# jamie8johnson/cqs

Measured on AMD Instinct MI355X. Metric: queries/sec @k=20 (brute-force cosine scan + top-k, 768-d fp32), higher is better.
Workload: dtype f32; 1 GPU; BASELINE configs[1]: 1000000 x 768 fp32 unit vectors, 1 query per step, brute-force cosine top-20; mode=single, rows_per_gpu=1000000, total_rows=1000000, dim=768, k=20, parallelism=single GPU, ranks_seen=1

## Files before the change

cqs_amd/csrc/index.hip:

```cpp
#include <hip/hip_runtime.h>

#include <algorithm>
#include <cstdio>
#include <cstdlib>
#include <cstring>
#include <new>

#include "abi_guard.h"
#include "roctx.h"
#include "index_internal.h"
#include "scan_bf16.h"
#include "scan_i8.h"
#include "search_host.h"

using cqs::kMaxK;
using cqs::kRowsPerBlock;

namespace cqs_idx {

uint64_t pad_rows(uint64_t n) { return (n + kRowsPerBlock - 1) / kRowsPerBlock * kRowsPerBlock; }

int32_t fail(cqs_hip_index* idx, int32_t code, const char* what, hipError_t e) {
    char buf[512];
    if (e != hipSuccess)
// ... 348 lines not shown
    if (x->done) hipEventDestroy(x->done);
    if (x->stream) hipStreamDestroy(x->stream);
    delete x;
} CQS_ABI_CATCH_VOID

uint64_t cqs_hip_index_len(const cqs_hip_index* x) CQS_ABI_TRY { return x ? (x->sh ? cqs_sharded::len(x) : x->n) : 0; } CQS_ABI_CATCH_VAL(0)
uint32_t cqs_hip_index_dim(const cqs_hip_index* x) CQS_ABI_TRY { return x ? x->dim : 0; } CQS_ABI_CATCH_VAL(0)
uint32_t cqs_hip_index_metric(const cqs_hip_index* x) CQS_ABI_TRY { return x ? x->metric : 0; } CQS_ABI_CATCH_VAL(0)
uint32_t cqs_hip_index_max_k(const cqs_hip_index* x) CQS_ABI_TRY { (void)x; return kMaxK; } CQS_ABI_CATCH_VAL(0)
int32_t cqs_hip_index_poisoned(const cqs_hip_index* x) CQS_ABI_TRY {
    if (x && x->sh) return cqs_sharded::poisoned(x);
    return x && x->poisoned.load(std::memory_order_acquire) ? 1 : 0;
} CQS_ABI_CATCH_NOHANDLE
int32_t cqs_hip_index_device(const cqs_hip_index* x) CQS_ABI_TRY { return x ? x->device : -1; } CQS_ABI_CATCH_NOHANDLE
uint64_t cqs_hip_index_row_base(const cqs_hip_index* x) CQS_ABI_TRY { return x ? x->row_base : 0; } CQS_ABI_CATCH_VAL(0)

size_t cqs_hip_index_last_error(const cqs_hip_index* x, char* buf, size_t cap) CQS_ABI_TRY {
    if (!x || !buf || cap == 0) return 0;
    std::lock_guard<std::mutex> g(x->mu);
    return cqs_search::copy_last_error(x->last_error.data(), x->last_error.size(), buf, cap);
} CQS_ABI_CATCH_VAL(0)

void cqs_hip_unpack_keys(const uint64_t* keys, size_t count, uint64_t* rows, float* scores) CQS_ABI_TRY {
    cqs_search::unpack_keys(keys, count, rows, scores);
} CQS_ABI_CATCH_VOID

size_t cqs_hip_merge_keys(const uint64_t* lists, const uint32_t* counts, size_t n_lists, size_t stride, size_t k,
                          uint64_t* out_keys) CQS_ABI_TRY {
    return cqs_search::merge_keys(lists, counts, n_lists, stride, k, out_keys);
} CQS_ABI_CATCH_VAL(0)

int32_t cqs_hip_index_search_device(cqs_hip_index* x, const float* d_queries, uint32_t b, uint32_t k,
                                    const uint32_t* d_keep_bitset, uint32_t mode, float threshold,
                                    uint64_t* d_out_keys, uint32_t* d_out_counts, void* stream) CQS_ABI_TRY {
    CQS_ROCTX_RANGE("cqs_hip_index_search_device");
    if (!x) return CQS_HIP_ERR_INVALID;
    if (x->sh) return CQS_HIP_ERR_INVALID;
    std::lock_guard<std::mutex> g(x->mu);
    if (x->poisoned.load(std::memory_order_acquire)) return CQS_HIP_ERR_POISONED;
    if (b == 0) return CQS_HIP_OK;
    if (!d_queries || !d_out_keys || !d_out_counts) return fail(x, CQS_HIP_ERR_INVALID, "search_device: null buffer");
    if (k == 0 || k > kMaxK) return fail(x, CQS_HIP_ERR_INVALID, "search_device: k out of range");
    if (mode > CQS_HIP_MODE_PIPELINE) return fail(x, CQS_HIP_ERR_INVALID, "search_device: bad mode");
    if (b > max_query_block(x)) return fail(x, CQS_HIP_ERR_INVALID, "search_device: batch exceeds scratch budget");
    HIP_TRY(x, hipSetDevice(x->device));
    hipStream_t st = (hipStream_t)stream;
    if (x->n == 0) {
        HIP_TRY(x, hipMemsetAsync(d_out_counts, 0, (size_t)b * sizeof(uint32_t), st));
        return CQS_HIP_OK;
    }
    int32_t rc = ensure_scratch(x, b, k);
    if (rc != CQS_HIP_OK) return rc;
    const uint32_t* gate = nullptr;
    if (shadow_takes(x, b, k, false) &&
        (rc = shadow_pass(x, d_queries, b, k, d_keep_bitset, mode, threshold, d_out_keys, d_out_counts, st, &gate)) != CQS_HIP_OK)
        return rc;
    return enqueue_search(x, d_queries, b, k, d_keep_bitset, mode, threshold, d_out_keys, d_out_counts, st, false, gate);
} CQS_ABI_CATCH(x)

}

namespace cqs_idx {

static void print_debug_stamps(cqs_hip_index* x) {
    unsigned long long h[16];
    if (hipMemcpy(h, x->d_dbg, sizeof h, hipMemcpyDeviceToHost) == hipSuccess)
        fprintf(stderr, "[cqs_hip] select_finish us: zero %.2f hist %.2f decide %.2f groups %.2f scores %.2f sort %.2f emit %.2f | groups=%llu cand=%llu\n",
                0.0, (h[1] - h[0]) / 100.0, (h[2] - h[1]) / 100.0, (h[3] - h[2]) / 100.0, (h[4] - h[3]) / 100.0,
                (h[5] - h[4]) / 100.0, (h[6] - h[5]) / 100.0, h[8], h[9]);
    std::vector<unsigned long long> w(2 * cqs::kDbgWaves);
    if (hipMemcpy(w.data(), x->d_dbg + 16, w.size() * sizeof(unsigned long long), hipMemcpyDeviceToHost) != hipSuccess) return;
    std::vector<double> st, en;
    unsigned long long t0 = ~0ull;
    for (uint32_t i = 0; i < cqs::kDbgWaves; ++i) if (w[2 * i] && w[2 * i] < t0) t0 = w[2 * i];
    for (uint32_t i = 0; i < cqs::kDbgWaves; ++i)
        if (w[2 * i] && w[2 * i + 1]) { st.push_back((w[2 * i] - t0) / 100.0); en.push_back((w[2 * i + 1] - t0) / 100.0); }
    if (!st.empty()) {
        std::sort(st.begin(), st.end());
        std::sort(en.begin(), en.end());
        auto pc = [](const std::vector<double>& v, double f) { return v[(size_t)(f * (v.size() - 1))]; };
        fprintf(stderr, "[cqs_hip] scan waves=%zu start us p0 %.1f p50 %.1f p90 %.1f p100 %.1f | end us p0 %.1f p10 %.1f p50 %.1f p90 %.1f p100 %.1f | select ends %.1f\n",
                st.size(), pc(st, 0), pc(st, .5), pc(st, .9), pc(st, 1), pc(en, 0), pc(en, .1), pc(en, .5), pc(en, .9), pc(en, 1),
                (h[6] - t0) / 100.0);
    }
    (void)hipMemset(x->d_dbg + 16, 0, w.size() * sizeof(unsigned long long));
}

static int32_t host_block(cqs_hip_index* x, const cqs_combine_req* const* qs, uint32_t nq, uint8_t* slots, uint32_t k,
                          const uint32_t* d_keep, uint32_t mode, float thr, bool gemv_only, std::vector<const cqs_combine_req*>* redo) {
    const KeepTab table{x->d_keep_tab, (uint32_t)x->keep_tab_stride, slots};
    const KeepTab* tab = slots ? &table : nullptr;
    HIP_TRY(x, hipMemcpyAsync(x->d_q, x->h_q, (size_t)nq * x->dim * sizeof(float), hipMemcpyHostToDevice, x->stream));
    const bool direct = x->h_out_keys_dev && x->h_out_counts_dev && (size_t)nq * k <= kDirectOutKeys;
    uint64_t* const keys = direct ? x->h_out_keys_dev : x->d_out_keys;
    uint32_t* const counts = direct ? x->h_out_counts_dev : x->d_out_counts;
    int32_t rc = redo ? shadow_pass(x, x->d_q, nq, k, d_keep, mode, thr, keys, counts, x->stream, nullptr, tab)
                      : enqueue_search(x, x->d_q, nq, k, d_keep, mode, thr, keys, counts, x->stream, gemv_only, nullptr, tab);
    if (rc != CQS_HIP_OK) return rc;
    if (redo) HIP_TRY(x, record_done(x, x->stream));
    if (!direct) {
        HIP_TRY(x, hipMemcpyAsync(x->h_out_keys, x->d_out_keys, (size_t)nq * k * sizeof(uint64_t), hipMemcpyDeviceToHost, x->stream));
        HIP_TRY(x, hipMemcpyAsync(x->h_out_counts, x->d_out_counts, (size_t)nq * sizeof(uint32_t), hipMemcpyDeviceToHost, x->stream));
    }
    const uint32_t* cert = nullptr;
    if (redo) HIP_TRY(x, shadow_verdicts(x, nq, &cert));
    HIP_TRY(x, hipStreamSynchronize(x->stream));
    if (!redo && x->d_dbg) print_debug_stamps(x);
    if (redo) redo->clear();
    uint64_t certified = 0;
// ... 251 lines not shown
```

cqs_amd/csrc/index_internal.h:

```cpp
#pragma once
#include <hip/hip_runtime.h>

#include <atomic>
#include <chrono>
#include <condition_variable>
#include <deque>
#include <mutex>
#include <string>
#include <vector>

#include "../../include/cqs_hip.h"
#include "scan_kernels.h"

namespace cqs_sharded { struct ShardSet; }
namespace cqs_idx { struct Shadow; }
namespace cqs_mmr { struct Scratch; }
namespace cqs_search { struct Args; }

struct cqs_combine_req {
    const float* q;
    uint32_t k, mode;
    float thr;
    uint64_t* out_rows;
    float* out_scores;
// ... 82 lines not shown

namespace cqs_idx {

constexpr size_t kMaxTimingEvents = 8192;
constexpr uint64_t kNtBytes = 200ull << 20;
constexpr uint32_t kGauxQueries = 32;
constexpr uint32_t kGauxMinK = 100;
constexpr uint32_t kCombineCap = 32;
constexpr size_t kDirectOutKeys = 8192;

uint64_t pad_rows(uint64_t n);
int32_t fail(cqs_hip_index* idx, int32_t code, const char* what, hipError_t e = hipSuccess);
void free_scratch(cqs_hip_index* x);
int32_t ensure_scratch(cqs_hip_index* x, uint32_t b, uint32_t k);
uint32_t max_query_block(const cqs_hip_index* x);
struct KeepTab { const uint32_t* d_tab; uint32_t stride; const uint8_t* slot; };
cqs::ScanArgs scan_args(const cqs_hip_index* x, const float* d_q, uint32_t b, uint32_t k, const uint32_t* d_keep,
                        uint32_t mode, float thr, size_t elem_bytes, bool gemv_only, void* dbg, const uint32_t* gate,
                        const KeepTab* tab = nullptr);
struct ShadowRows { const uint16_t* bf16; const int8_t* i8; const float* i8_scale; const float* bq; };
int32_t scan_select(cqs_hip_index* x, const cqs::ScanArgs& a, hipStream_t st, const ShadowRows* shadow,
                    uint64_t* out_keys, uint32_t* out_counts);
inline hipError_t order_after_last(cqs_hip_index* x, hipStream_t st) {
    return x->done_valid && x->done_stream != st ? hipStreamWaitEvent(st, x->done, 0) : hipSuccess;
}
inline hipError_t record_done(cqs_hip_index* x, hipStream_t st) {
    const hipError_t e = hipEventRecord(x->done, st);
    if (e == hipSuccess) { x->done_stream = st; x->done_valid = true; }
    return e;
}
int32_t enqueue_search(cqs_hip_index* x, const float* d_q, uint32_t b, uint32_t k, const uint32_t* d_keep,
                       uint32_t mode, float thr, uint64_t* d_out_keys, uint32_t* d_out_counts, hipStream_t st,
                       bool gemv_only = false, const uint32_t* gate = nullptr, const KeepTab* tab = nullptr);
hipError_t quiesce(cqs_hip_index* x);
int32_t create_owned(const float* rows, uint64_t n, uint32_t dim, uint32_t metric, int32_t device, uint64_t row_base,
                     cqs_hip_index** out);
int32_t stage_keep(cqs_hip_index* x, const uint32_t* host_words, uint64_t words);
int32_t ensure_keep(cqs_hip_index* x, uint64_t words);
bool ensure_keep_tab(cqs_hip_index* x);
void free_keep_tab(cqs_hip_index* x);
int32_t create_common(uint64_t n, uint32_t dim, uint32_t metric, int32_t device, uint64_t row_base,
                      cqs_hip_index** out, cqs_hip_index** made);
void read_combine_env(cqs_hip_index* x);
int32_t shadow_auto(cqs_hip_index* x);
int32_t shadow_extend(cqs_hip_index* x, uint64_t n_old);
void shadow_free(cqs_hip_index* x);
struct ShadowBuffers { uint16_t* bf16; int8_t* i8; float* i8_scale; };
ShadowBuffers shadow_buffers(const cqs_hip_index* x);
bool shadow_takes(const cqs_hip_index* x, uint32_t b, uint32_t k, bool gemv_only);
bool shadow_uses_i8(const cqs_hip_index* x, uint32_t b, uint32_t k);
int32_t shadow_pass(cqs_hip_index* x, const float* d_q, uint32_t nb, uint32_t k, const uint32_t* d_keep, uint32_t mode,
                    float thr, uint64_t* out_keys, uint32_t* out_counts, hipStream_t st, const uint32_t** device_gate,
                    const KeepTab* tab = nullptr);
hipError_t shadow_verdicts(cqs_hip_index* x, uint32_t nb, const uint32_t** h_cert);

bool search_planned(cqs_hip_index* x, const cqs_search::Args& a, int32_t* rc);
std::vector<cqs_combine_req> requests(const cqs_search::Args& a, float thr);
int32_t injected_failure(cqs_hip_index* x);
int32_t search_blocks_locked(cqs_hip_index* x, const cqs_combine_req* qs, uint32_t b, uint32_t k_eff, const uint32_t* d_keep,
                             uint32_t mode, float threshold, bool gemv_only);
void tags_free(cqs_hip_index* x);
void tags_regrow(cqs_hip_index* x);

int32_t search_host_locked(cqs_hip_index* x, const cqs_combine_req* qs, uint32_t b, uint32_t k, const uint32_t* keep_bitset,
                           uint32_t mode, float threshold, bool gemv_only);
int32_t search_filtered_locked(cqs_hip_index* x, const cqs_combine_req* qs, uint32_t b, uint32_t k, uint32_t mode, float threshold);
int32_t combine_search(cqs_hip_index* x, cqs_combine_req& r);

struct Segment { int device; float* d_rows; uint64_t rows; hipStream_t stream; };
int32_t save_segments(cqs_hip_index* err_owner, const std::vector<Segment>& segs, uint32_t dim, uint32_t metric,
                      const char* path, uint64_t* out_checksum);
int32_t open_blob(const char* path, uint32_t expected_dim, uint64_t expected_rows, int* fd_out, uint64_t* rows,
                  uint32_t* metric, uint64_t* checksum);
int32_t read_blob_into(int fd, uint64_t checksum, uint32_t dim, const std::vector<Segment>& segs);

}

namespace cqs_mmr {
void free_scratch(cqs_hip_index* x);
int32_t run(cqs_hip_index* owner, hipStream_t st, const float* src, const uint32_t* h_idx, const float* h_scores, uint32_t m,
            uint32_t limit, float lambda, float* out_gram, uint32_t* out_picks);
int32_t gather_rows(cqs_hip_index* c, const uint32_t* h_idx, uint32_t mc, const float** out_block);
int32_t staging(cqs_hip_index* parent, uint32_t m, float** out_block);
}

namespace cqs_sharded {
int32_t pairwise(cqs_hip_index* parent, const uint64_t* cand_rows, uint32_t m, float* out);
int32_t mmr(cqs_hip_index* parent, const uint64_t* cand_rows, const float* cand_scores, uint32_t m, uint32_t limit,
            float lambda, uint32_t* out_picks, uint32_t* out_count);
void destroy(cqs_hip_index* parent);
int32_t search(cqs_hip_index* parent, const float* queries, uint32_t b, uint32_t query_dim, uint32_t k,
               const uint32_t* keep_bitset, uint32_t mode, float threshold, uint64_t* out_rows, float* out_scores,
               uint32_t* out_counts);
int32_t search_combined(cqs_hip_index* parent, cqs_combine_req* const* batch, uint32_t nb);
int32_t neighbors(cqs_hip_index* parent, uint64_t target_row, uint32_t limit, uint64_t* out_rows, float* out_scores,
                  uint32_t* out_count);
int32_t extend(cqs_hip_index* parent, const float* rows, uint64_t n_new);
int32_t save(cqs_hip_index* parent, const char* path, uint64_t* out_checksum);
uint64_t len(const cqs_hip_index* parent);
int32_t poisoned(const cqs_hip_index* parent);
void set_timing(cqs_hip_index* parent, int32_t enable);
int32_t scan_time(cqs_hip_index* parent, uint32_t* launches, double* total_ms);
}

#define HIP_TRY(idx, expr)                                                        \
    do {                                                                          \
// ... 5 lines not shown
```

cqs_amd/csrc/index_shadow.hip:

```cpp
#include <cstdlib>
#include <cstring>
#include <new>

#include "abi_guard.h"
#include "index_internal.h"
#include "scan_bf16.h"
#include "scan_i8.h"

namespace cqs_idx {

constexpr uint64_t kShadowAutoBytes = 1ull << 30;
constexpr uint64_t kShadowFreeMinBytes = 4ull << 30;
constexpr double kShadowFreeFrac = 0.10;
constexpr uint32_t kStatWords = 10, kStatCounts = 3, kStatI8 = 5, kStatI8Counts = 8;

struct Shadow {
    uint16_t* d_bf16 = nullptr;
    uint64_t cap = 0;
    int8_t* d_i8 = nullptr;
    float* d_i8_scale = nullptr;
    double r8 = 0.0, norm8 = 0.0;
    double r = 0.0;
    double norm = 0.0;
    unsigned long long* d_stats = nullptr;
    uint64_t* d_ekeys = nullptr;
    uint32_t* d_cert = nullptr;
    float* d_bq = nullptr;
    uint32_t* d_tickets = nullptr;
    uint32_t* h_cert = nullptr;
    uint32_t* h_cert_dev = nullptr;
};

static void shadow_device_counts(cqs_hip_index* x, uint32_t first, uint64_t* certified, uint64_t* fallbacks) {
    unsigned long long c[2];
    if (!x->shadow || !x->shadow->d_stats || quiesce(x) != hipSuccess) return;
    hipError_t e = hipMemcpyAsync(c, x->shadow->d_stats + first, sizeof c, hipMemcpyDeviceToHost, x->stream);
    if (e == hipSuccess) e = hipStreamSynchronize(x->stream);
    if (e != hipSuccess) { (void)hipGetLastError(); return; }
    *certified += c[0];
    *fallbacks += c[1];
}

static void i8_free(Shadow* s) {
    hipFree(s->d_i8); hipFree(s->d_i8_scale);
    s->d_i8 = nullptr; s->d_i8_scale = nullptr;
}

void shadow_free(cqs_hip_index* x) {
    Shadow* s = x->shadow;
    if (!s) return;
    uint64_t c = 0, f = 0;
    shadow_device_counts(x, kStatCounts, &c, &f);
    x->stat_certified.fetch_add(c, std::memory_order_relaxed);
    x->stat_fallbacks.fetch_add(f, std::memory_order_relaxed);
    c = f = 0;
    shadow_device_counts(x, kStatI8Counts, &c, &f);
    x->stat_i8_certified.fetch_add(c, std::memory_order_relaxed);
    x->stat_i8_fallbacks.fetch_add(f, std::memory_order_relaxed);
    i8_free(s);
    hipFree(s->d_bf16); hipFree(s->d_stats); hipFree(s->d_ekeys);
    hipFree(s->d_cert); hipFree(s->d_bq); hipFree(s->d_tickets); hipHostFree(s->h_cert);
    delete s;
    x->shadow = nullptr;
}

ShadowBuffers shadow_buffers(const cqs_hip_index* x) {
    const Shadow* s = x->shadow;
    return s ? ShadowBuffers{s->d_bf16, s->d_i8, s->d_i8_scale} : ShadowBuffers{nullptr, nullptr, nullptr};
}

static int32_t shadow_convert(cqs_hip_index* x, uint64_t row0, bool* outlier) {
    Shadow* s = x->shadow;
    HIP_TRY(x, hipMemsetAsync(s->d_stats + 2, 0, sizeof(unsigned long long), x->stream));
    HIP_TRY(x, cqs::launch_shadow_build(x->d_rows, s->d_bf16, row0, x->n - row0, x->dim, cqs::shadow_gamma(x->dim),
                                        s->d_stats, x->stream));
    unsigned long long st[3];
    HIP_TRY(x, hipMemcpyAsync(st, s->d_stats, sizeof st, hipMemcpyDeviceToHost, x->stream));
    HIP_TRY(x, hipStreamSynchronize(x->stream));
    double r, m;
    memcpy(&r, &st[0], sizeof r);
    memcpy(&m, &st[1], sizeof m);
    s->r = r * (1.0 + 0x1p-30);
    s->norm = m * (1.0 + 0x1p-30);
    *outlier = st[2] != 0;
    return CQS_HIP_OK;
}

static int32_t i8_convert(cqs_hip_index* x, uint64_t row0) {
    Shadow* s = x->shadow;
    HIP_TRY(x, cqs::launch_i8_build(x->d_rows, s->d_i8, s->d_i8_scale, row0, x->n - row0, x->dim, cqs::i8_gamma(x->dim),
                                    s->d_stats + kStatI8, x->stream));
    unsigned long long st[2];
    HIP_TRY(x, hipMemcpyAsync(st, s->d_stats + kStatI8, sizeof st, hipMemcpyDeviceToHost, x->stream));
    HIP_TRY(x, hipStreamSynchronize(x->stream));
    double r, m;
    memcpy(&r, &st[0], sizeof r);
    memcpy(&m, &st[1], sizeof m);
    s->r8 = r * (1.0 + 0x1p-30);
    s->norm8 = m * (1.0 + 0x1p-30);
    return CQS_HIP_OK;
}

static uint64_t i8_bytes(uint64_t cap, uint32_t dim) { return cap * dim + cap * sizeof(float); }

static int32_t i8_enable(cqs_hip_index* x, bool* built) {
    Shadow* s = x->shadow;
    *built = false;
    if (hipMalloc(&s->d_i8, (size_t)s->cap * x->dim) != hipSuccess ||
        hipMalloc(&s->d_i8_scale, (size_t)s->cap * sizeof(float)) != hipSuccess) {
        (void)hipGetLastError();
        i8_free(s);
        return CQS_HIP_OK;
    }
    const int32_t rc = i8_convert(x, 0);
// ... 22 lines not shown
            int8_t* n8 = nullptr;
            float* ns = nullptr;
            if (hipMalloc(&n8, (size_t)x->cap_rows * x->dim) != hipSuccess || hipMalloc(&ns, (size_t)x->cap_rows * sizeof(float)) != hipSuccess) {
                (void)hipGetLastError();
                hipFree(n8);
                i8_free(s);
                x->last_error = "extend: no device memory to grow the int8 copy of the shadow; int8 copy turned off";
            } else {
                e = hipMemcpyAsync(n8, s->d_i8, (size_t)n_old * x->dim, hipMemcpyDeviceToDevice, x->stream);
                if (e == hipSuccess) e = hipMemcpyAsync(ns, s->d_i8_scale, (size_t)n_old * sizeof(float), hipMemcpyDeviceToDevice, x->stream);
                if (e == hipSuccess) e = hipStreamSynchronize(x->stream);
                if (e != hipSuccess) { hipFree(n8); hipFree(ns); return fail(x, CQS_HIP_ERR_DEVICE, "extend: int8 copy", e); }
                i8_free(s);
                s->d_i8 = n8;
                s->d_i8_scale = ns;
            }
        }
        s->cap = x->cap_rows;
    }
    bool outlier = false;
    int32_t rc = shadow_convert(x, n_old, &outlier);
    if (rc == CQS_HIP_OK && s->d_i8 && !outlier) rc = i8_convert(x, n_old);
    if (rc != CQS_HIP_OK) return rc;
    if (outlier) {
        shadow_free(x);
        x->last_error = "extend: a new row has a component of magnitude >= 2^64; bf16 shadow turned off";
    }
    return CQS_HIP_OK;
}

static bool dim_ok(uint32_t dim) { return dim % 8u == 0u && dim <= cqs::kShadowMaxDim; }
static const char* const kDimRule = ": dim must be a multiple of 8 and <= 2048";

static int32_t shadow_enable(cqs_hip_index* x, const char* what) {
    std::string pre(what);
    if (!dim_ok(x->dim)) return fail(x, CQS_HIP_ERR_INVALID, (pre + kDimRule).c_str());
    if (x->shadow) return CQS_HIP_OK;
    auto oom = [&](hipError_t e) { (void)hipGetLastError(); shadow_free(x); return fail(x, CQS_HIP_ERR_NOMEM, (pre + ": allocation").c_str(), e); };
    Shadow* s = x->shadow = new (std::nothrow) Shadow();
    if (!s) return oom(hipErrorOutOfMemory);
    const uint64_t cap = x->cap_rows ? x->cap_rows : 1;
    hipError_t e;
    if ((e = hipMalloc(&s->d_bf16, (size_t)cap * x->dim * sizeof(uint16_t))) != hipSuccess) return oom(e);
    s->cap = cap;
    unsigned long long* stats = nullptr;
    if ((e = hipMalloc(&stats, kStatWords * sizeof(unsigned long long))) != hipSuccess) return oom(e);
    if ((e = hipMemsetAsync(stats, 0, kStatWords * sizeof(unsigned long long), x->stream)) != hipSuccess) { hipFree(stats); return oom(e); }
    s->d_stats = stats;
    if ((e = hipMalloc(&s->d_ekeys, (size_t)cqs::kShadowMaxQ * (cqs::kMaxK - 1) * sizeof(uint64_t))) != hipSuccess) return oom(e);
    if ((e = hipMalloc(&s->d_cert, (size_t)cqs::kShadowMaxQ * sizeof(uint32_t))) != hipSuccess) return oom(e);
    if ((e = hipMalloc(&s->d_bq, (size_t)cqs::kShadowMaxQ * sizeof(float))) != hipSuccess) return oom(e);
    if ((e = hipMalloc(&s->d_tickets, (size_t)cqs::kShadowMaxQ * sizeof(uint32_t))) != hipSuccess) return oom(e);
    if ((e = hipMemsetAsync(s->d_tickets, 0, (size_t)cqs::kShadowMaxQ * sizeof(uint32_t), x->stream)) != hipSuccess) return oom(e);
    if ((e = hipHostMalloc(&s->h_cert, (size_t)cqs::kShadowMaxQ * sizeof(uint32_t), hipHostMallocDefault)) != hipSuccess) return oom(e);
    if (hipHostGetDevicePointer((void**)&s->h_cert_dev, s->h_cert, 0) != hipSuccess) {
        (void)hipGetLastError();
        s->h_cert_dev = nullptr;
    }
    bool outlier = false;
    const int32_t rc = shadow_convert(x, 0, &outlier);
    if (rc != CQS_HIP_OK) { shadow_free(x); return rc; }
    if (outlier) {
        shadow_free(x);
        return fail(x, CQS_HIP_ERR_INVALID, (pre + ": a finite row has a component of magnitude >= 2^64").c_str());
    }
    return CQS_HIP_OK;
}

static bool i8_dim_ok(uint32_t dim) { return cqs::i8_dim_ok(dim); }
static const char* const kI8DimRule = ": dim must be a multiple of 16 and <= 2048";
static int32_t i8_auto(cqs_hip_index* x) {
    Shadow* s = x->shadow;
    if (!s || s->d_i8) return CQS_HIP_OK;
    const char* env = getenv("CQS_HIP_SCAN_I8");
    if (env && env[0] == '0') return CQS_HIP_OK;
    if (!(env && env[0] == '1') && x->n * x->dim * sizeof(float) < kShadowAutoBytes) return CQS_HIP_OK;
    const std::string pre("int8 copy of the shadow not built (the bf16 copy serves every block)");
    if (!i8_dim_ok(x->dim)) { x->last_error = pre + kI8DimRule; return CQS_HIP_OK; }
    size_t free_b = 0, total_b = 0;
    if (hipMemGetInfo(&free_b, &total_b) != hipSuccess) {
        (void)hipGetLastError();
        x->last_error = pre + ": hipMemGetInfo failed";
        return CQS_HIP_OK;
    }
    const uint64_t need = i8_bytes(s->cap, x->dim);
    const uint64_t frac = (uint64_t)(kShadowFreeFrac * (double)total_b);
    const uint64_t reserve = frac > kShadowFreeMinBytes ? frac : kShadowFreeMinBytes;
    bool built = false;
    if (free_b >= need && free_b - need >= reserve) {
        const int32_t rc = i8_enable(x, &built);
        if (rc != CQS_HIP_OK) return rc;
    }
    if (!built) x->last_error = pre + ": the device would keep less than max(4 GiB, 10 %) of its memory free with both copies";
    return CQS_HIP_OK;
}

int32_t shadow_auto(cqs_hip_index* x) {
    const char* env = getenv("CQS_HIP_SCAN_BF16");
    if (env && env[0] == '0') return CQS_HIP_OK;
    const bool any_size = env && env[0] == '1';
    const uint64_t f32_bytes = x->n * x->dim * sizeof(float);
    if (!any_size && f32_bytes < kShadowAutoBytes) {
        x->last_error = "bf16 shadow not built: f32 corpus below 1 GiB (CQS_HIP_SCAN_BF16=1 builds it at any size)";
        return CQS_HIP_OK;
    }
    if (!dim_ok(x->dim)) {
        x->last_error = std::string("bf16 shadow not built") + kDimRule;
        return CQS_HIP_OK;
    }
    size_t free_b = 0, total_b = 0;
    if (hipMemGetInfo(&free_b, &total_b) != hipSuccess) {
        (void)hipGetLastError();
        x->last_error = "bf16 shadow not built: hipMemGetInfo failed";
        return CQS_HIP_OK;
    }
    const uint64_t cap = x->cap_rows ? x->cap_rows : 1;
    const uint64_t need = cap * x->dim * sizeof(uint16_t) + (cqs::kMaxK + 2ull) * cqs::kShadowMaxQ * sizeof(uint64_t);
    const uint64_t frac = (uint64_t)(kShadowFreeFrac * (double)total_b);
    const uint64_t reserve = frac > kShadowFreeMinBytes ? frac : kShadowFreeMinBytes;
    if (free_b < need || free_b - need < reserve) {
        x->last_error = "bf16 shadow not built: the device would keep less than max(4 GiB, 10 %) of its memory free";
        return CQS_HIP_OK;
    }
    int32_t rc = shadow_enable(x, "bf16 shadow not built");
    if (rc == CQS_HIP_OK) rc = i8_auto(x);
    return rc == CQS_HIP_ERR_DEVICE ? rc : CQS_HIP_OK;
}

bool shadow_takes(const cqs_hip_index* x, uint32_t b, uint32_t k, bool gemv_only) {
    return x->shadow && b <= cqs::kShadowMaxQ && (gemv_only || !cqs::use_mfma(b, x->dim)) && cqs::shadow_kprime(k) >= k;
}

bool shadow_uses_i8(const cqs_hip_index* x, uint32_t b, uint32_t k) {
    return x->shadow && x->shadow->d_i8 && b <= cqs::kI8MaxQ && cqs::i8_k_ok(k);
}

int32_t shadow_pass(cqs_hip_index* x, const float* d_q, uint32_t nb, uint32_t k, const uint32_t* d_keep, uint32_t mode,
                    float threshold, uint64_t* out_keys, uint32_t* out_counts, hipStream_t st, const uint32_t** device_gate,
                    const KeepTab* tab) {
    const Shadow* s = x->shadow;
    uint32_t* const cert = device_gate || !s->h_cert_dev ? s->d_cert : s->h_cert_dev;
    if (device_gate) *device_gate = cert;
    if (device_gate) HIP_TRY(x, order_after_last(x, st));
    const bool i8 = shadow_uses_i8(x, nb, k);
    const uint32_t kp = i8 ? cqs::i8_kprime(k) : cqs::shadow_kprime(k);
    const double r_max = i8 ? s->r8 : s->r, norm_max = i8 ? s->norm8 : s->norm;
    const bool bound_first = mode == CQS_HIP_MODE_PIPELINE;
    if (bound_first) {
        if (i8) HIP_TRY(x, cqs::launch_i8_bound(d_q, nb, x->dim, r_max, norm_max, s->d_bq, st));
        else HIP_TRY(x, cqs::launch_shadow_bound(d_q, nb, x->dim, r_max, norm_max, s->d_bq, st));
    }
    const cqs::ScanArgs a = scan_args(x, d_q, nb, kp + 1u, d_keep, mode, threshold, i8 ? sizeof(int8_t) : sizeof(uint16_t), true, nullptr, nullptr, tab);
    const ShadowRows rows{i8 ? nullptr : s->d_bf16, i8 ? s->d_i8 : nullptr, s->d_i8_scale, s->d_bq};
    const int32_t rc = scan_select(x, a, st, &rows, nullptr, nullptr);
    if (rc == CQS_HIP_OK)
        HIP_TRY(x, cqs::launch_rescore_certify(a, (uint32_t)x->row_base, k, kp, bound_first ? 0u : (i8 ? 2u : 1u), r_max, norm_max,
                                               s->d_bq, s->d_tickets, s->d_ekeys, out_keys, out_counts, cert,
                                               device_gate ? s->d_stats + kStatCounts : nullptr,
                                               device_gate && i8 ? s->d_stats + kStatI8Counts : nullptr, st));
    return rc;
}

hipError_t shadow_verdicts(cqs_hip_index* x, uint32_t nb, const uint32_t** h_cert) {
    const Shadow* s = x->shadow;
    *h_cert = s->h_cert;
    return s->h_cert_dev ? hipSuccess : hipMemcpyAsync(s->h_cert, s->d_cert, (size_t)nb * sizeof(uint32_t), hipMemcpyDeviceToHost, x->stream);
}

}

using namespace cqs_idx;

extern "C" {

int32_t cqs_hip_index_set_bf16_scan(cqs_hip_index* x, int32_t enable) CQS_ABI_TRY {
    if (!x || x->sh) return CQS_HIP_ERR_INVALID;
    std::lock_guard<std::mutex> g(x->mu);
    if (x->poisoned.load(std::memory_order_acquire)) return CQS_HIP_ERR_POISONED;
    HIP_TRY(x, hipSetDevice(x->device));
    HIP_TRY(x, quiesce(x));
    if (!enable) { shadow_free(x); return CQS_HIP_OK; }
    if (x->borrow) return fail(x, CQS_HIP_ERR_INVALID, "set_bf16_scan: index borrows its rows (they may change under the bound)");
    const int32_t rc = shadow_enable(x, "set_bf16_scan");
    return rc == CQS_HIP_OK ? i8_auto(x) : rc;
} CQS_ABI_CATCH(x)

void cqs_hip_index_bf16_stats(const cqs_hip_index* x, uint64_t* bytes, uint64_t* certified, uint64_t* fallbacks) CQS_ABI_TRY {
    uint64_t by = 0, c = 0, f = 0;
    if (x && !x->sh) {
        cqs_hip_index* m = const_cast<cqs_hip_index*>(x);
        std::lock_guard<std::mutex> g(m->mu);
        by = m->shadow ? m->shadow->cap * m->dim * sizeof(uint16_t) : 0;
        c = m->stat_certified.load(std::memory_order_relaxed);
        f = m->stat_fallbacks.load(std::memory_order_relaxed);
        if (m->shadow && hipSetDevice(m->device) == hipSuccess) shadow_device_counts(m, kStatCounts, &c, &f);
    }
    if (bytes) *bytes = by;
    if (certified) *certified = c;
    if (fallbacks) *fallbacks = f;
} CQS_ABI_CATCH_VOID

void cqs_hip_index_i8_stats(const cqs_hip_index* x, uint64_t* bytes, uint64_t* certified, uint64_t* fallbacks) CQS_ABI_TRY {
    uint64_t by = 0, c = 0, f = 0;
    if (x && !x->sh) {
        cqs_hip_index* m = const_cast<cqs_hip_index*>(x);
        std::lock_guard<std::mutex> g(m->mu);
        by = m->shadow && m->shadow->d_i8 ? i8_bytes(m->shadow->cap, m->dim) : 0;
        c = m->stat_i8_certified.load(std::memory_order_relaxed);
        f = m->stat_i8_fallbacks.load(std::memory_order_relaxed);
        if (m->shadow && hipSetDevice(m->device) == hipSuccess) shadow_device_counts(m, kStatI8Counts, &c, &f);
    }
    if (bytes) *bytes = by;
    if (certified) *certified = c;
// ... 135 lines not shown
```

cqs_amd/csrc/scan_bf16.hip:

```cpp
#include "scan_bf16.h"
#include "scan_i8.h"
#include "launch_util.h"
#include "rank_sort.h"
#include "scan_gemv_device.h"
#include "select_device.h"

namespace cqs {

static_assert(kShadowKMax == kMaxK, "shadow k' policy and the select agree on max k");

typedef __bf16 bf2 __attribute__((ext_vector_type(2)));

__device__ __forceinline__ float bf_lo(uint32_t w) { return __uint_as_float(w << 16); }
__device__ __forceinline__ float bf_hi(uint32_t w) { return __uint_as_float(w & 0xFFFF0000u); }
__device__ __forceinline__ float key_score(uint64_t key) {
    const uint32_t ok = (uint32_t)(key >> 32);
    return __uint_as_float((ok & 0x80000000u) ? (ok ^ 0x80000000u) : ~ok);
}

__global__ __launch_bounds__(256) void shadow_build_kernel(const float* __restrict__ rows, uint16_t* __restrict__ shadow,
                                                           uint64_t row0, uint64_t n_rows, uint32_t dim, double gamma,
                                                           unsigned long long* __restrict__ stats) {
    const int lane = threadIdx.x & 63;
    const uint64_t waves = (uint64_t)gridDim.x * (blockDim.x >> 6);
    for (uint64_t r = (uint64_t)blockIdx.x * (blockDim.x >> 6) + (threadIdx.x >> 6); r < n_rows; r += waves) {
        const float* xp = rows + (row0 + r) * dim;
        uint16_t* op = shadow + (row0 + r) * dim;
        double d2 = 0.0, n2 = 0.0, t2 = 0.0;
        bool fin = true, big = false;
        for (uint32_t i = (uint32_t)lane * 2u; i < dim; i += 128u) {
            const f2 v = *(const f2*)(xp + i);
            const bf2 h = __builtin_convertvector(v, bf2);
            const uint32_t w = __builtin_bit_cast(uint32_t, h);
            *(uint32_t*)(op + i) = w;
            const float t0 = bf_lo(w), t1 = bf_hi(w);
            fin = fin && __builtin_isfinite(v.x) && __builtin_isfinite(v.y);
            big = big || __builtin_fabsf(v.x) >= 0x1p64f || __builtin_fabsf(v.y) >= 0x1p64f;
            const double e0 = (double)v.x - (double)t0, e1 = (double)v.y - (double)t1;
            d2 += e0 * e0 + e1 * e1;
            n2 += (double)v.x * (double)v.x + (double)v.y * (double)v.y;
            t2 += (double)t0 * (double)t0 + (double)t1 * (double)t1;
        }
#pragma unroll
        for (int m = 32; m >= 1; m >>= 1) {
            d2 += __shfl_xor(d2, m, 64);
            n2 += __shfl_xor(n2, m, 64);
            t2 += __shfl_xor(t2, m, 64);
        }
        const bool all_fin = __ballot(!fin) == 0ull;
        const bool any_big = __ballot(big) != 0ull;
        if (lane == 0 && all_fin) {
            const double nx = sqrt(n2), nt = sqrt(t2);
            const double rb = sqrt(d2) + gamma * (nx + nt);
            atomicMax(&stats[0], (unsigned long long)__double_as_longlong(rb));
// ... 286 lines not shown
    float* bq;
    uint32_t* tickets;
    uint32_t bound;
    double r_max, norm_max;
    uint64_t* out_keys;
    uint32_t* out_counts;
    uint32_t* cert;
    unsigned long long* counters;
    unsigned long long* counters2;
};

constexpr uint32_t kTailWaves = 16;

template <int NCH>
__global__ __launch_bounds__(1024) void rescore_certify_kernel(const TailParams p) {
    __shared__ uint64_t s_keys[kShadowKMax];
    __shared__ uint64_t s_sorted[kShadowKMax];
    __shared__ __attribute__((aligned(16))) uint32_t s_ok[kShadowKMax + 4];
    __shared__ uint32_t s_cnt, s_flag, s_last;
    const uint32_t lane = threadIdx.x & 63u;
    const uint32_t qi = blockIdx.y;
    const uint32_t wave = (uint32_t)__builtin_amdgcn_readfirstlane((int)(blockIdx.x * kTailWaves + (threadIdx.x >> 6)));
    const uint32_t n_waves = gridDim.x * kTailWaves;
    const uint32_t dim = p.dim;
    const float* qp = p.q + (size_t)qi * dim;
    if (threadIdx.x == 0) s_cnt = 0u;
    if (qi == 0u && blockIdx.x == 0u)
        for (uint32_t i = threadIdx.x; i < kWorkWords; i += 1024u) p.work[i] = 0u;

    const uint32_t n_tasks = p.tiers.total();
    uint32_t found;
    const uint64_t* akeys = select_body(p.scores + (size_t)qi * p.n_pad, p.gmax + (size_t)qi * n_tasks,
                                        p.gaux ? p.gaux + (size_t)qi * n_tasks : nullptr, p.n_pad, p.tiers, p.kprime + 1u,
                                        p.row_base, p.bins, nullptr, found);
    const uint32_t ac = found < p.kprime + 1u ? found : p.kprime + 1u;
    const uint32_t nc = ac < p.kprime ? ac : p.kprime;
    const uint64_t key_next = ac > p.kprime ? akeys[p.kprime] : 0ull;

    for (uint32_t slot = wave; slot <= nc; slot += n_waves) {
        if (slot == 0u) {
            if (p.bound != 0u) {
                const float v = p.bound == 2u ? wave_i8_bound(qp, dim, p.r_max, p.norm_max, lane)
                                              : wave_shadow_bound(qp, dim, p.r_max, p.norm_max, lane);
                if (lane == 0u)
                    __hip_atomic_store((uint32_t*)p.bq + qi, __float_as_uint(v), __ATOMIC_RELAXED, __HIP_MEMORY_SCOPE_AGENT);
            }
            continue;
        }
        const uint32_t i = slot - 1u;
        const uint64_t key = akeys[i];
        const uint32_t grow = 0xFFFFFFFFu - (uint32_t)key;
        const float* rp = p.rows + (size_t)(grow - p.row_base) * dim;
        f4 x[NCH], qv[NCH];
#pragma unroll
        for (int c = 0; c < NCH; ++c) {
            const uint32_t idx = (uint32_t)c * 256u + lane * 4u;
            const bool in = idx < dim;
            const uint32_t off = in ? idx : dim - 4u;
            x[c] = *(const f4*)(rp + off);
            const f4 v = *(const f4*)(qp + off);
            qv[c] = in ? v : (f4)(0.f);
        }
        f2 acc2 = (f2)(0.f);
#pragma unroll
        for (int c = 0; c < NCH; ++c) {
            const f2 xlo = __builtin_shufflevector(x[c], x[c], 0, 1);
            const f2 xhi = __builtin_shufflevector(x[c], x[c], 2, 3);
            acc2 = __builtin_elementwise_fma(xlo, __builtin_shufflevector(qv[c], qv[c], 0, 1), acc2);
            acc2 = __builtin_elementwise_fma(xhi, __builtin_shufflevector(qv[c], qv[c], 2, 3), acc2);
        }
        float s = acc2.x + acc2.y;
#pragma unroll
        for (int m = 32; m >= 1; m >>= 1) s += __shfl_xor(s, m, 64);
        bool keep = __builtin_fabsf(s) <= 3.4028234664e38f;
        if (keep && p.mode == 1u) {
            s = s < 0.f ? 0.f : (s > 1.f ? 1.f : s);
            keep = s >= p.thr;
        }
        if (lane == 0u)
            __hip_atomic_store(p.ekeys + (size_t)qi * p.kprime + i, keep ? pack_key(okey(s), grow) : 0ull, __ATOMIC_RELAXED,
                               __HIP_MEMORY_SCOPE_AGENT);
    }
    asm volatile("s_waitcnt vmcnt(0)" ::: "memory");
    __syncthreads();
    if (threadIdx.x == 0) {
        const uint32_t t = __hip_atomic_fetch_add(p.tickets + qi, 1u, __ATOMIC_RELAXED, __HIP_MEMORY_SCOPE_AGENT);
        const bool last = t == gridDim.x - 1u;
        if (last) __hip_atomic_store(p.tickets + qi, 0u, __ATOMIC_RELAXED, __HIP_MEMORY_SCOPE_AGENT);
        s_last = last ? 1u : 0u;
    }
    __syncthreads();
    if (s_last == 0u) return;

    if (threadIdx.x < nc) {
        const uint64_t key = __hip_atomic_load(p.ekeys + (size_t)qi * p.kprime + threadIdx.x, __ATOMIC_RELAXED, __HIP_MEMORY_SCOPE_AGENT);
        if (key != 0ull) s_keys[atomicAdd(&s_cnt, 1u)] = key;
    }
    __syncthreads();
    const uint32_t m = s_cnt;
    rank_sort_keys(s_keys, m, s_sorted, s_ok, &s_flag);
    const uint32_t k = p.k;
    const uint32_t outc = m < k ? m : k;
    for (uint32_t i = threadIdx.x; i < k; i += 1024u) p.out_keys[(size_t)qi * k + i] = (i < outc) ? s_sorted[i] : 0ull;
    if (threadIdx.x == 0) {
        p.out_counts[qi] = outc;
        const float bq = __uint_as_float(__hip_atomic_load((uint32_t*)p.bq + qi, __ATOMIC_RELAXED, __HIP_MEMORY_SCOPE_AGENT));
        bool ok = false;
        if (__builtin_fabsf(bq) <= 3.4028234664e38f) {
            if (ac <= p.kprime) ok = true;
            else if (m >= k) {
                float t = key_score(key_next) + bq;
                if (p.mode == 1u) t = t < 0.f ? 0.f : (t > 1.f ? 1.f : t);
                ok = t < key_score(s_sorted[k - 1u]);
            }
        }
        p.cert[qi] = ok ? 1u : 0u;
        if (p.counters) atomicAdd(&p.counters[ok ? 0 : 1], 1ull);
        if (p.counters2) atomicAdd(&p.counters2[ok ? 0 : 1], 1ull);
    }
}

#ifndef CQS_TAIL_MAX_BLOCKS_PER_CU
#define CQS_TAIL_MAX_BLOCKS_PER_CU 1u
#endif

hipError_t launch_rescore_certify(const ScanArgs& a, uint32_t row_base, uint32_t k, uint32_t kprime, uint32_t bound,
                                  double r_max, double norm_max, float* bq, uint32_t* tickets, uint64_t* ekeys,
                                  uint64_t* out_keys, uint32_t* out_counts, uint32_t* cert, unsigned long long* counters,
                                  unsigned long long* counters2, hipStream_t st) {
    const uint32_t b = a.b, dim = a.dim;
    if (b == 0) return hipSuccess;
// ... 26 lines not shown
```

Measured before the change: 6645 queries/s.

## Add single-launch fused f32 scan+top-k fallback after shadow pass

When the bf16/i8 shadow pass is used with a device gate, the uncertified fallback now goes through one new kernel. That kernel scans all fp32 rows per CU, keeps per-block candidate lists in LDS with periodic rank-sort cuts, and merges across blocks with a ticketed last-block reduction. This replaces the multi-kernel enqueue_search path and is meant to cut launch count and global scratch traffic. It adds a persistent global list buffer and tickets, can be disabled with an environment variable, and moves the shared f32 dot helpers into a header.

```diff
diff --git a/cqs_amd/csrc/f32_score.h b/cqs_amd/csrc/f32_score.h
--- /dev/null
+++ b/cqs_amd/csrc/f32_score.h
@@ -0,0 +1,56 @@
+#pragma once
+#include "scan_device.h"
+
+namespace cqs {
+
+template <int NCH, bool NT = false>
+__device__ __forceinline__ void f32_row_fragments(const float* rp, uint32_t dim, uint32_t lane, f4 (&x)[NCH]) {
+#pragma unroll
+    for (int c = 0; c < NCH; ++c) {
+        const uint32_t idx = (uint32_t)c * 256u + lane * 4u;
+        const uint32_t off = idx < dim ? idx : dim - 4u;
+        if (NT) x[c] = __builtin_nontemporal_load((const f4*)(rp + off));
+        else x[c] = *(const f4*)(rp + off);
+    }
+}
+
+template <int NCH>
+__device__ __forceinline__ void f32_fragments(const float* rp, const float* qp, uint32_t dim, uint32_t lane, f4 (&x)[NCH],
+                                              f4 (&qv)[NCH]) {
+#pragma unroll
+    for (int c = 0; c < NCH; ++c) {
+        const uint32_t idx = (uint32_t)c * 256u + lane * 4u;
+        const bool in = idx < dim;
+        const uint32_t off = in ? idx : dim - 4u;
+        x[c] = *(const f4*)(rp + off);
+        const f4 v = *(const f4*)(qp + off);
+        qv[c] = in ? v : (f4)(0.f);
+    }
+}
+
+template <int NCH>
+__device__ __forceinline__ float f32_dot_chain(const f4 (&x)[NCH], const f4 (&qv)[NCH]) {
+    f2 acc2 = (f2)(0.f);
+#pragma unroll
+    for (int c = 0; c < NCH; ++c) {
+        const f2 xlo = __builtin_shufflevector(x[c], x[c], 0, 1);
+        const f2 xhi = __builtin_shufflevector(x[c], x[c], 2, 3);
+        acc2 = __builtin_elementwise_fma(xlo, __builtin_shufflevector(qv[c], qv[c], 0, 1), acc2);
+        acc2 = __builtin_elementwise_fma(xhi, __builtin_shufflevector(qv[c], qv[c], 2, 3), acc2);
+    }
+    float s = acc2.x + acc2.y;
+#pragma unroll
+    for (int m = 32; m >= 1; m >>= 1) s += __shfl_xor(s, m, 64);
+    return s;
+}
+
+__device__ __forceinline__ bool f32_emit(float& s, uint32_t mode, float thr) {
+    bool keep = __builtin_fabsf(s) <= 3.4028234664e38f;
+    if (keep && mode == 1u) {
+        s = s < 0.f ? 0.f : (s > 1.f ? 1.f : s);
+        keep = s >= thr;
+    }
+    return keep;
+}
+
+}
diff --git a/cqs_amd/csrc/index.hip b/cqs_amd/csrc/index.hip
--- a/cqs_amd/csrc/index.hip
+++ b/cqs_amd/csrc/index.hip
@@ -424,9 +424,13 @@
     int32_t rc = ensure_scratch(x, b, k);
     if (rc != CQS_HIP_OK) return rc;
     const uint32_t* gate = nullptr;
-    if (shadow_takes(x, b, k, false) &&
-        (rc = shadow_pass(x, d_queries, b, k, d_keep_bitset, mode, threshold, d_out_keys, d_out_counts, st, &gate)) != CQS_HIP_OK)
-        return rc;
+    if (shadow_takes(x, b, k, false)) {
+        if ((rc = shadow_pass(x, d_queries, b, k, d_keep_bitset, mode, threshold, d_out_keys, d_out_counts, st, &gate)) != CQS_HIP_OK)
+            return rc;
+        bool taken = false;
+        rc = shadow_fallback(x, d_queries, b, k, d_keep_bitset, mode, threshold, d_out_keys, d_out_counts, st, gate, &taken);
+        if (rc != CQS_HIP_OK || taken) return rc;
+    }
     return enqueue_search(x, d_queries, b, k, d_keep_bitset, mode, threshold, d_out_keys, d_out_counts, st, false, gate);
 } CQS_ABI_CATCH(x)
 
diff --git a/cqs_amd/csrc/index_internal.h b/cqs_amd/csrc/index_internal.h
--- a/cqs_amd/csrc/index_internal.h
+++ b/cqs_amd/csrc/index_internal.h
@@ -158,6 +158,8 @@
 int32_t shadow_pass(cqs_hip_index* x, const float* d_q, uint32_t nb, uint32_t k, const uint32_t* d_keep, uint32_t mode,
                     float thr, uint64_t* out_keys, uint32_t* out_counts, hipStream_t st, const uint32_t** device_gate,
                     const KeepTab* tab = nullptr);
+int32_t shadow_fallback(cqs_hip_index* x, const float* d_q, uint32_t nb, uint32_t k, const uint32_t* d_keep, uint32_t mode,
+                        float thr, uint64_t* out_keys, uint32_t* out_counts, hipStream_t st, const uint32_t* gate, bool* taken);
 hipError_t shadow_verdicts(cqs_hip_index* x, uint32_t nb, const uint32_t** h_cert);
 
 bool search_planned(cqs_hip_index* x, const cqs_search::Args& a, int32_t* rc);
diff --git a/cqs_amd/csrc/index_shadow.hip b/cqs_amd/csrc/index_shadow.hip
--- a/cqs_amd/csrc/index_shadow.hip
+++ b/cqs_amd/csrc/index_shadow.hip
@@ -5,6 +5,7 @@
 #include "abi_guard.h"
 #include "index_internal.h"
 #include "scan_bf16.h"
+#include "scan_fallback.h"
 #include "scan_i8.h"
 
 namespace cqs_idx {
@@ -27,6 +28,9 @@
     uint32_t* d_cert = nullptr;
     float* d_bq = nullptr;
     uint32_t* d_tickets = nullptr;
+    uint64_t* d_fb_lists = nullptr;
+    uint32_t* d_fb_tickets = nullptr;
+    bool fb_one_launch = true;
     uint32_t* h_cert = nullptr;
     uint32_t* h_cert_dev = nullptr;
 };
@@ -59,7 +63,8 @@
     x->stat_i8_fallbacks.fetch_add(f, std::memory_order_relaxed);
     i8_free(s);
     hipFree(s->d_bf16); hipFree(s->d_stats); hipFree(s->d_ekeys);
-    hipFree(s->d_cert); hipFree(s->d_bq); hipFree(s->d_tickets); hipHostFree(s->h_cert);
+    hipFree(s->d_cert); hipFree(s->d_bq); hipFree(s->d_tickets); hipFree(s->d_fb_lists); hipFree(s->d_fb_tickets);
+    hipHostFree(s->h_cert);
     delete s;
     x->shadow = nullptr;
 }
@@ -188,6 +193,11 @@
     if ((e = hipMalloc(&s->d_bq, (size_t)cqs::kShadowMaxQ * sizeof(float))) != hipSuccess) return oom(e);
     if ((e = hipMalloc(&s->d_tickets, (size_t)cqs::kShadowMaxQ * sizeof(uint32_t))) != hipSuccess) return oom(e);
     if ((e = hipMemsetAsync(s->d_tickets, 0, (size_t)cqs::kShadowMaxQ * sizeof(uint32_t), x->stream)) != hipSuccess) return oom(e);
+    const char* fb_env = getenv("CQS_HIP_FALLBACK_ONE_LAUNCH");
+    s->fb_one_launch = !(fb_env && fb_env[0] == '0');
+    if ((e = hipMalloc(&s->d_fb_lists, cqs::f32_topk_fallback_words(x->n_cu) * sizeof(uint64_t))) != hipSuccess) return oom(e);
+    if ((e = hipMalloc(&s->d_fb_tickets, (size_t)cqs::kMaxGemvQ * sizeof(uint32_t))) != hipSuccess) return oom(e);
+    if ((e = hipMemsetAsync(s->d_fb_tickets, 0, (size_t)cqs::kMaxGemvQ * sizeof(uint32_t), x->stream)) != hipSuccess) return oom(e);
     if ((e = hipHostMalloc(&s->h_cert, (size_t)cqs::kShadowMaxQ * sizeof(uint32_t), hipHostMallocDefault)) != hipSuccess) return oom(e);
     if (hipHostGetDevicePointer((void**)&s->h_cert_dev, s->h_cert, 0) != hipSuccess) {
         (void)hipGetLastError();
@@ -251,7 +261,8 @@
         return CQS_HIP_OK;
     }
     const uint64_t cap = x->cap_rows ? x->cap_rows : 1;
-    const uint64_t need = cap * x->dim * sizeof(uint16_t) + (cqs::kMaxK + 2ull) * cqs::kShadowMaxQ * sizeof(uint64_t);
+    const uint64_t need = cap * x->dim * sizeof(uint16_t) + (cqs::kMaxK + 2ull) * cqs::kShadowMaxQ * sizeof(uint64_t) +
+                          cqs::f32_topk_fallback_words(x->n_cu) * sizeof(uint64_t);
     const uint64_t frac = (uint64_t)(kShadowFreeFrac * (double)total_b);
     const uint64_t reserve = frac > kShadowFreeMinBytes ? frac : kShadowFreeMinBytes;
     if (free_b < need || free_b - need < reserve) {
@@ -295,6 +306,20 @@
                                                device_gate ? s->d_stats + kStatCounts : nullptr,
                                                device_gate && i8 ? s->d_stats + kStatI8Counts : nullptr, st));
     return rc;
+}
+
+int32_t shadow_fallback(cqs_hip_index* x, const float* d_q, uint32_t nb, uint32_t k, const uint32_t* d_keep, uint32_t mode,
+                        float threshold, uint64_t* out_keys, uint32_t* out_counts, hipStream_t st, const uint32_t* gate,
+                        bool* taken) {
+    const Shadow* s = x->shadow;
+    *taken = false;
+    if (!s || !gate || !s->fb_one_launch) return CQS_HIP_OK;
+    const cqs::ScanArgs a = scan_args(x, d_q, nb, k, d_keep, mode, threshold, sizeof(float), false, nullptr, gate);
+    if (!cqs::f32_topk_fallback_takes(a)) return CQS_HIP_OK;
+    HIP_TRY(x, cqs::launch_f32_topk_fallback(a, (uint32_t)x->row_base, gate, s->d_fb_lists, s->d_fb_tickets, out_keys, out_counts, st));
+    HIP_TRY(x, record_done(x, st));
+    *taken = true;
+    return CQS_HIP_OK;
 }
 
 hipError_t shadow_verdicts(cqs_hip_index* x, uint32_t nb, const uint32_t** h_cert) {
diff --git a/cqs_amd/csrc/scan_bf16.hip b/cqs_amd/csrc/scan_bf16.hip
--- a/cqs_amd/csrc/scan_bf16.hip
+++ b/cqs_amd/csrc/scan_bf16.hip
@@ -1,5 +1,6 @@
 #include "scan_bf16.h"
 #include "scan_i8.h"
+#include "f32_score.h"
 #include "launch_util.h"
 #include "rank_sort.h"
 #include "scan_gemv_device.h"
@@ -392,31 +393,9 @@
         const uint32_t grow = 0xFFFFFFFFu - (uint32_t)key;
         const float* rp = p.rows + (size_t)(grow - p.row_base) * dim;
         f4 x[NCH], qv[NCH];
-#pragma unroll
-        for (int c = 0; c < NCH; ++c) {
-            const uint32_t idx = (uint32_t)c * 256u + lane * 4u;
-            const bool in = idx < dim;
-            const uint32_t off = in ? idx : dim - 4u;
-            x[c] = *(const f4*)(rp + off);
-            const f4 v = *(const f4*)(qp + off);
-            qv[c] = in ? v : (f4)(0.f);
-        }
-        f2 acc2 = (f2)(0.f);
-#pragma unroll
-        for (int c = 0; c < NCH; ++c) {
-            const f2 xlo = __builtin_shufflevector(x[c], x[c], 0, 1);
-            const f2 xhi = __builtin_shufflevector(x[c], x[c], 2, 3);
-            acc2 = __builtin_elementwise_fma(xlo, __builtin_shufflevector(qv[c], qv[c], 0, 1), acc2);
-            acc2 = __builtin_elementwise_fma(xhi, __builtin_shufflevector(qv[c], qv[c], 2, 3), acc2);
-        }
-        float s = acc2.x + acc2.y;
-#pragma unroll
-        for (int m = 32; m >= 1; m >>= 1) s += __shfl_xor(s, m, 64);
-        bool keep = __builtin_fabsf(s) <= 3.4028234664e38f;
-        if (keep && p.mode == 1u) {
-            s = s < 0.f ? 0.f : (s > 1.f ? 1.f : s);
-            keep = s >= p.thr;
-        }
+        f32_fragments<NCH>(rp, qp, dim, lane, x, qv);
+        float s = f32_dot_chain<NCH>(x, qv);
+        const bool keep = f32_emit(s, p.mode, p.thr);
         if (lane == 0u)
             __hip_atomic_store(p.ekeys + (size_t)qi * p.kprime + i, keep ? pack_key(okey(s), grow) : 0ull, __ATOMIC_RELAXED,
                                __HIP_MEMORY_SCOPE_AGENT);
diff --git a/cqs_amd/csrc/scan_fallback.h b/cqs_amd/csrc/scan_fallback.h
--- /dev/null
+++ b/cqs_amd/csrc/scan_fallback.h
@@ -0,0 +1,18 @@
+#pragma once
+#include "scan_kernels.h"
+
+namespace cqs {
+
+constexpr uint32_t kFallbackMaxK = 128;
+
+inline size_t f32_topk_fallback_words(uint32_t n_cu) { return (size_t)kMaxGemvQ * n_cu * kFallbackMaxK; }
+
+inline bool f32_topk_fallback_takes(const ScanArgs& a) {
+    return a.b >= 1u && a.b <= kMaxGemvQ && a.k >= 1u && a.k <= kFallbackMaxK && !a.keep_tab && a.dim >= 8u &&
+           a.dim % 4u == 0u && a.dim <= 2048u && a.n >= 1u && a.n <= 0xFFFF0000u;
+}
+
+hipError_t launch_f32_topk_fallback(const ScanArgs& a, uint32_t row_base, const uint32_t* gate, uint64_t* lists,
+                                    uint32_t* tickets, uint64_t* out_keys, uint32_t* out_counts, hipStream_t st);
+
+}
diff --git a/cqs_amd/csrc/scan_fallback.hip b/cqs_amd/csrc/scan_fallback.hip
--- /dev/null
+++ b/cqs_amd/csrc/scan_fallback.hip
@@ -0,0 +1,211 @@
+#include "scan_fallback.h"
+#include "f32_score.h"
+#include "launch_util.h"
+#include "rank_sort.h"
+
+namespace cqs {
+
+constexpr uint32_t kFbThreads = 1024;
+constexpr uint32_t kFbWaveRows = 16;
+constexpr uint32_t kFbTileRows = (kFbThreads / 64u) * kFbWaveRows;
+constexpr uint32_t kFbBuf = 768;
+static_assert(kFallbackMaxK + kFbTileRows <= kFbBuf && kFbBuf <= kFbThreads, "a cut list plus one tile fits the buffer and the sort");
+
+struct FallbackParams {
+    const float* rows;
+    const float* q;
+    uint32_t n, dim, b, k, mode, row_base;
+    float thr;
+    const uint32_t* keep;
+    const uint32_t* gate;
+    uint64_t* lists;
+    uint32_t* tickets;
+    uint64_t* out_keys;
+    uint32_t* out_counts;
+};
+
+struct FallbackLds {
+    uint64_t* sorted;
+    uint32_t* ok;
+    uint64_t* thr;
+    uint32_t* cnt;
+    uint32_t* last;
+    uint32_t* flag;
+    float* q;
+    uint64_t* keys;
+};
+constexpr size_t kFbLdsFixed = kFbBuf * 8u + (kFbBuf + 4u) * 4u + kMaxGemvQ * 8u + kMaxGemvQ * 4u + kMaxGemvQ * 4u + 16u;
+static_assert(kFbLdsFixed % 16u == 0u, "the per-query arrays start 16-byte aligned");
+inline size_t fallback_lds_bytes(uint32_t b, uint32_t nch) { return kFbLdsFixed + (size_t)b * (nch * 1024u + kFbBuf * 8u); }
+
+__device__ __forceinline__ FallbackLds carve_lds(unsigned char* base, uint32_t b, uint32_t qwords) {
+    FallbackLds l;
+    l.sorted = (uint64_t*)base;                  base += kFbBuf * 8u;
+    l.ok = (uint32_t*)base;                      base += (kFbBuf + 4u) * 4u;
+    l.thr = (uint64_t*)base;                     base += kMaxGemvQ * 8u;
+    l.cnt = (uint32_t*)base;                     base += kMaxGemvQ * 4u;
+    l.last = (uint32_t*)base;                    base += kMaxGemvQ * 4u;
+    l.flag = (uint32_t*)base;                    base += 16u;
+    l.q = (float*)base;                          base += (size_t)b * qwords * 4u;
+    l.keys = (uint64_t*)base;
+    return l;
+}
+
+__device__ __forceinline__ void cut_list(const FallbackLds& l, uint32_t qi, uint32_t k) {
+    uint64_t* keys = l.keys + (size_t)qi * kFbBuf;
+    const uint32_t m = l.cnt[qi];
+    rank_sort_keys(keys, m, l.sorted, l.ok, l.flag);
+    const uint32_t kept = m < k ? m : k;
+    if (threadIdx.x < kept) keys[threadIdx.x] = l.sorted[threadIdx.x];
+    if (threadIdx.x == 0) {
+        l.cnt[qi] = kept;
+        l.thr[qi] = kept == k ? l.sorted[k - 1u] : 0ull;
+    }
+    __syncthreads();
+}
+
+__device__ __forceinline__ uint32_t lists_to_cut(const FallbackLds& l, uint32_t b) {
+    __syncthreads();
+    uint32_t need = 0u;
+    for (uint32_t qi = 0; qi < b; ++qi) need |= (l.cnt[qi] > kFbBuf - kFbTileRows ? 1u : 0u) << qi;
+    __syncthreads();
+    return (uint32_t)__builtin_amdgcn_readfirstlane((int)need);
+}
+
+template <int NCH, bool NT>
+__global__ __launch_bounds__(1024) void f32_topk_fallback_kernel(const FallbackParams p) {
+    if (gate_closed(p.gate, p.b)) return;
+    extern __shared__ __attribute__((aligned(16))) unsigned char s_fb[];
+    constexpr uint32_t QW = (uint32_t)NCH * 256u;
+    constexpr int RI = NCH <= 4 ? 4 : (NCH <= 6 ? 2 : 1);
+    const uint32_t b = p.b, k = p.k, n = p.n, dim = p.dim;
+    const FallbackLds l = carve_lds(s_fb, b, QW);
+    const uint32_t lane = threadIdx.x & 63u;
+    const uint32_t wave = (uint32_t)__builtin_amdgcn_readfirstlane((int)(threadIdx.x >> 6));
+
+    for (uint32_t i = threadIdx.x; i < b * QW; i += kFbThreads) {
+        const uint32_t qi = i / QW, d = i % QW;
+        l.q[i] = d < dim ? p.q[(size_t)qi * dim + d] : 0.f;
+    }
+    if (threadIdx.x < kMaxGemvQ) { l.cnt[threadIdx.x] = 0u; l.thr[threadIdx.x] = 0ull; l.last[threadIdx.x] = 0u; }
+    __syncthreads();
+
+    const uint32_t last_row = n - 1u;
+    const uint32_t n_tiles = (n + kFbTileRows - 1u) / kFbTileRows;
+    for (uint32_t tile = blockIdx.x; tile < n_tiles; tile += gridDim.x) {
+        const uint32_t row0 = tile * kFbTileRows + wave * kFbWaveRows;
+        uint32_t mask = 0u;
+        if (row0 < n) {
+            const uint32_t left = n - row0;
+            mask = left >= kFbWaveRows ? 0xFFFFu : (1u << left) - 1u;
+            if (p.keep) mask &= p.keep[row0 >> 5] >> (row0 & 31u);
+        }
+        mask = (uint32_t)__builtin_amdgcn_readfirstlane((int)mask);
+        for (uint32_t j = 0; j < kFbWaveRows / (uint32_t)RI; ++j) {
+            const uint32_t m = (mask >> ((uint32_t)RI * j)) & ((1u << RI) - 1u);
+            if (m == 0u) continue;
+            const uint32_t r0 = row0 + (uint32_t)RI * j;
+            f4 x[RI][NCH];
+#pragma unroll
+            for (int r = 0; r < RI; ++r) {
+                const uint32_t row = r0 + (uint32_t)r > last_row ? last_row : r0 + (uint32_t)r;
+                f32_row_fragments<NCH, NT>(p.rows + (size_t)row * dim, dim, lane, x[r]);
+            }
+            for (uint32_t qi = 0; qi < b; ++qi) {
+                f4 qv[NCH];
+#pragma unroll
+                for (int c = 0; c < NCH; ++c) qv[c] = *(const f4*)(l.q + qi * QW + (uint32_t)c * 256u + lane * 4u);
+#pragma unroll
+                for (int r = 0; r < RI; ++r) {
+                    float s = f32_dot_chain<NCH>(x[r], qv);
+                    const bool emit = f32_emit(s, p.mode, p.thr);
+                    if (lane == 0u && ((m >> r) & 1u) && emit) {
+                        const uint64_t key = pack_key(okey(s), p.row_base + r0 + (uint32_t)r);
+                        if (key > l.thr[qi]) l.keys[(size_t)qi * kFbBuf + atomicAdd(&l.cnt[qi], 1u)] = key;
+                    }
+                }
+            }
+        }
+        const uint32_t need = lists_to_cut(l, b);
+        for (uint32_t qi = 0; qi < b; ++qi)
+            if ((need >> qi) & 1u) cut_list(l, qi, k);
+    }
+
+    __syncthreads();
+    for (uint32_t qi = 0; qi < b; ++qi) {
+        cut_list(l, qi, k);
+        if (threadIdx.x < k)
+            __hip_atomic_store(p.lists + ((size_t)qi * gridDim.x + blockIdx.x) * k + threadIdx.x,
+                               threadIdx.x < l.cnt[qi] ? l.keys[(size_t)qi * kFbBuf + threadIdx.x] : 0ull, __ATOMIC_RELAXED,
+                               __HIP_MEMORY_SCOPE_AGENT);
+    }
+    asm volatile("s_waitcnt vmcnt(0)" ::: "memory");
+    __syncthreads();
+    if (threadIdx.x < b) {
+        const uint32_t t = __hip_atomic_fetch_add(p.tickets + threadIdx.x, 1u, __ATOMIC_RELAXED, __HIP_MEMORY_SCOPE_AGENT);
+        l.last[threadIdx.x] = t == gridDim.x - 1u ? 1u : 0u;
+    }
+    __syncthreads();
+
+    for (uint32_t qi = 0; qi < b; ++qi) {
+        if (l.last[qi] == 0u) continue;
+        if (threadIdx.x == 0) { l.cnt[qi] = 0u; l.thr[qi] = 0ull; }
+        __syncthreads();
+        const uint64_t* lists = p.lists + (size_t)qi * gridDim.x * k;
+        const uint32_t total = gridDim.x * k;
+        for (uint32_t c0 = 0; c0 < total; c0 += kFbThreads) {
+            const uint32_t idx = c0 + threadIdx.x;
+            const uint64_t key = idx < total ? __hip_atomic_load(lists + idx, __ATOMIC_RELAXED, __HIP_MEMORY_SCOPE_AGENT) : 0ull;
+            for (uint32_t step = 0; step < kFbThreads / kFbTileRows; ++step) {
+                if (threadIdx.x / kFbTileRows == step && key > l.thr[qi])
+                    l.keys[(size_t)qi * kFbBuf + atomicAdd(&l.cnt[qi], 1u)] = key;
+                if ((lists_to_cut(l, b) >> qi) & 1u) cut_list(l, qi, k);
+            }
+        }
+        cut_list(l, qi, k);
+        const uint32_t outc = l.cnt[qi];
+        for (uint32_t i = threadIdx.x; i < k; i += kFbThreads)
+            p.out_keys[(size_t)qi * k + i] = i < outc ? l.keys[(size_t)qi * kFbBuf + i] : 0ull;
+        if (threadIdx.x == 0) {
+            p.out_counts[qi] = outc;
+            __hip_atomic_store(p.tickets + qi, 0u, __ATOMIC_RELAXED, __HIP_MEMORY_SCOPE_AGENT);
+        }
+    }
+}
+
+hipError_t launch_f32_topk_fallback(const ScanArgs& a, uint32_t row_base, const uint32_t* gate, uint64_t* lists,
+                                    uint32_t* tickets, uint64_t* out_keys, uint32_t* out_counts, hipStream_t st) {
+    if (!f32_topk_fallback_takes(a) || !gate || !lists || !tickets || a.n_cu == 0u) return hipErrorInvalidValue;
+    const FallbackParams p{a.rows, a.q, a.n, a.dim, a.b, a.k, a.mode, row_base, a.threshold, a.keep, gate, lists, tickets,
+                           out_keys, out_counts};
+    const uint32_t nch = (a.dim + 255u) / 256u;
+    const uint32_t n_tiles = (a.n + kFbTileRows - 1u) / kFbTileRows;
+    const dim3 grid(n_tiles < a.n_cu ? n_tiles : a.n_cu), block(kFbThreads);
+    const size_t lds = fallback_lds_bytes(a.b, nch);
+    auto launch = [&](auto nch_c, auto nt_c) -> hipError_t {
+        auto kern = f32_topk_fallback_kernel<decltype(nch_c)::value, decltype(nt_c)::value>;
+        if (lds > 48u * 1024u) {
+            static DynLdsOnce once;
+            const hipError_t e = once.ensure((const void*)kern, lds);
+            if (e != hipSuccess) return e;
+        }
+        hipLaunchKernelGGL(kern, grid, block, lds, st, p);
+        return hipGetLastError();
+    };
+    auto by_nt = [&](auto nch_c) -> hipError_t {
+        return a.nontemporal ? launch(nch_c, std::true_type{}) : launch(nch_c, std::false_type{});
+    };
+    switch (nch) {
+        case 1: return by_nt(std::integral_constant<int, 1>{});
+        case 2: return by_nt(std::integral_constant<int, 2>{});
+        case 3: return by_nt(std::integral_constant<int, 3>{});
+        case 4: return by_nt(std::integral_constant<int, 4>{});
+        case 5: return by_nt(std::integral_constant<int, 5>{});
+        case 6: return by_nt(std::integral_constant<int, 6>{});
+        case 7: return by_nt(std::integral_constant<int, 7>{});
+        case 8: return by_nt(std::integral_constant<int, 8>{});
+        default: return hipErrorInvalidValue;
+    }
+}
+
+}
```

After: 6720 queries/s (median of 6 runs). 1.1% higher.
